# shanghong/Multiband-RF-pulse-Design

Hardware: AMD Instinct MI355X
Metric: FIR designs/sec, n=512 taps m=16384 arbitrary-phase SOCP (fir_ap_cvx form) (higher is better)
Workload: dtype f64

## Files before the change

### include/mbfir.h

```cpp
#ifndef MBFIR_H
#define MBFIR_H

#ifdef __cplusplus
extern "C" {
#endif

#define MBFIR_SOLVED 0
#define MBFIR_INFEASIBLE 1
#define MBFIR_NUMERICAL 2
#define MBFIR_EARLY_FAIL 3
#define MBFIR_E_ARG (-1)
#define MBFIR_E_HIP (-2)
#define MBFIR_E_NODEVICE (-3)

typedef struct mbfir_ctx mbfir_ctx;

typedef struct mbfir_opts {
    int grid_m;
    int max_iter;
    double feastol;
    double abstol;
    double reltol;
    int refine;
    int verbose;
// ... 3 lines not shown
    int ddkkt;
    int lanes;
} mbfir_opts;

typedef struct mbfir_info {
    int status;
    int iters;
    int n_unknowns;
    int n_rows;
    int n_freq;
    int n_lp, n_q3, n_big;
    double pcost, dcost, gap, relgap, pres, dres;
    double ms_assemble, ms_solve, ms_post, ms_total;
    double ms_gram;
    double ms_chol;
    double gram_flop;
    int gram_launches;
    int lattice;
    double chol_flop;
    int chol_launches;
    int builds;
    int dd_iters;
    int dd_kmax;
    int collectives;
    int lanes;
    int dd_form;
    double ms_cap;
    double cap_flop;
    double collective_bytes;
    int correctors;
    int correctors_taken;
    int gv_passes;
    int gtv_passes;
} mbfir_info;

typedef int (*mbfir_allreduce_fn)(void* buf, long count, int op, void* user);

int  mbfir_comm_unique_id(mbfir_ctx* ctx, char* id128);
int  mbfir_comm_init(mbfir_ctx* ctx, int nranks, int rank, const char* id128);
void mbfir_comm_destroy(mbfir_ctx* ctx);
int  mbfir_test_comm_allreduce(mbfir_ctx* ctx, double* v, long n, int op);

mbfir_ctx*  mbfir_create(int device_id);
void        mbfir_destroy(mbfir_ctx* ctx);
const char* mbfir_last_error(mbfir_ctx* ctx);
void        mbfir_default_opts(mbfir_opts* opts);
void        mbfir_set_allreduce(mbfir_ctx* ctx, mbfir_allreduce_fn fn, void* user);
const char* mbfir_version(void);

int mbfir_ap_solve(mbfir_ctx* ctx, int n, int nband, const double* f, const double* a,
                   const double* d, double obj, double peak, const mbfir_opts* opts,
                   double* h_re, double* h_im, mbfir_info* info);

int mbfir_qp_solve(mbfir_ctx* ctx, int n, int nband, const double* f, const double* a,
                   const double* d, double kquad, const double* obj, int nobj,
                   const mbfir_opts* opts, double* h_re, double* h_im, mbfir_info* info);

int mbfir_linprog_solve(mbfir_ctx* ctx, int n, int nband, const double* f, const double* a,
                        const double* d, const mbfir_opts* opts,
                        double* h_re, double* h_im, mbfir_info* info);

int mbfir_qprog_phs_solve(mbfir_ctx* ctx, int n, int nband, const double* f,
                          const double* ac_re, const double* ac_im,
                          const double* dc_re, const double* dc_im, const mbfir_opts* opts,
                          double* h_re, double* h_im, mbfir_info* info);

// ... 121 lines not shown
```

### multiband-rf-pulse-design_amd/__init__.py

```python
import ctypes as C
import os

import numpy as np

_HERE = os.path.dirname(os.path.abspath(__file__))
LIB_PATH = os.path.join(_HERE, "libmbfir.so")

SOLVED, INFEASIBLE, NUMERICAL, EARLY_FAIL = 0, 1, 2, 3
E_ARG, E_HIP, E_NODEVICE = -1, -2, -3


class MbfirError(RuntimeError):
    pass


class Opts(C.Structure):
    _fields_ = [("grid_m", C.c_int), ("max_iter", C.c_int), ("feastol", C.c_double),
                ("abstol", C.c_double), ("reltol", C.c_double), ("refine", C.c_int),
                ("verbose", C.c_int), ("shard_rank", C.c_int), ("shard_size", C.c_int),
                ("dense_trig", C.c_int), ("ddkkt", C.c_int), ("lanes", C.c_int)]


class Info(C.Structure):
    _fields_ = [("status", C.c_int), ("iters", C.c_int), ("n_unknowns", C.c_int), ("n_rows", C.c_int),
                ("n_freq", C.c_int), ("n_lp", C.c_int), ("n_q3", C.c_int), ("n_big", C.c_int),
                ("pcost", C.c_double), ("dcost", C.c_double), ("gap", C.c_double), ("relgap", C.c_double),
                ("pres", C.c_double), ("dres", C.c_double),
                ("ms_assemble", C.c_double), ("ms_solve", C.c_double), ("ms_post", C.c_double),
                ("ms_total", C.c_double), ("ms_gram", C.c_double), ("ms_chol", C.c_double),
                ("gram_flop", C.c_double), ("gram_launches", C.c_int), ("lattice", C.c_int),
                ("chol_flop", C.c_double), ("chol_launches", C.c_int), ("builds", C.c_int),
                ("dd_iters", C.c_int), ("dd_kmax", C.c_int), ("collectives", C.c_int), ("lanes", C.c_int),
                ("dd_form", C.c_int), ("ms_cap", C.c_double), ("cap_flop", C.c_double),
                ("collective_bytes", C.c_double), ("correctors", C.c_int), ("correctors_taken", C.c_int),
                ("gv_passes", C.c_int), ("gtv_passes", C.c_int)]

    def as_dict(self):
        return {k: getattr(self, k) for k, _ in self._fields_}


class Job(C.Structure):
    _fields_ = [("which", C.c_int), ("n", C.c_int), ("nband", C.c_int), ("rc", C.c_int),
                ("f", C.POINTER(C.c_double)), ("a", C.POINTER(C.c_double)), ("d", C.POINTER(C.c_double)),
                ("params", C.c_double * 4), ("h_re", C.POINTER(C.c_double)), ("h_im", C.POINTER(C.c_double)),
                ("info", Info), ("z", C.POINTER(C.c_double)), ("z_cap", C.c_int), ("err", C.c_char * 128)]


class RemezJob(C.Structure):
    _fields_ = [("numtaps", C.c_int), ("nband", C.c_int), ("type", C.c_int), ("edges", C.POINTER(C.c_double)),
                ("desired", C.POINTER(C.c_double)), ("weight", C.POINTER(C.c_double)), ("h", C.POINTER(C.c_double)),
                ("ext", C.POINTER(C.c_double)), ("status", C.c_int), ("iterations", C.c_int), ("delta", C.c_double)]


class RemezOpts(C.Structure):
    _fields_ = [("grid_density", C.c_int), ("maxiter", C.c_int)]


ALLREDUCE_FN = C.CFUNCTYPE(C.c_int, C.c_void_p, C.c_long, C.c_int, C.c_void_p)

_dp = C.POINTER(C.c_double)
_ip = C.POINTER(C.c_int)
_lp = C.POINTER(C.c_long)
_lib = None

SYMBOLS = {
    "mbfir_create": (C.c_void_p, [C.c_int]),
    "mbfir_destroy": (None, [C.c_void_p]),
    "mbfir_last_error": (C.c_char_p, [C.c_void_p]),
# ... 1119 lines not shown
```

### multiband-rf-pulse-design_amd/csrc/api.cpp

```cpp
#include "../../include/mbfir.h"
#include "program.h"
#include "pulse.h"
#include "solver.h"
#include <chrono>
#include <cmath>
#include <cstdio>
#include <algorithm>
#include <cstdlib>
#include <cstring>
#include <functional>
#include <atomic>
#include <condition_variable>
#include <map>
#include <mutex>
#include <memory>
#include <system_error>
#include <thread>

using namespace mbfir;

struct mbfir_ctx {
    std::unique_ptr<Solver> solver;
    int device = 0;
    std::vector<double> last_x;
// ... 30 lines not shown
    s.shard_size = o->shard_size;
    s.dense_trig = o->dense_trig != 0;
    return s;
}

int status_to_rc(int st) {
    switch (st) {
        case ST_OPTIMAL:
        case ST_OPTIMAL_INACCURATE: return MBFIR_SOLVED;
        case ST_PRIMAL_INFEASIBLE:
        case ST_DUAL_INFEASIBLE: return MBFIR_INFEASIBLE;
        default: return MBFIR_NUMERICAL;
    }
}

void fill_info(mbfir_info* info, const TrigProgram& P, const SolveInfo& si, int rc, double t0, double t_asm,
               double t_solved, double t_end) {
    if (!info) return;
    std::memset(info, 0, sizeof(*info));
    info->status = rc; info->iters = si.iters; info->n_unknowns = P.N();
    info->n_rows = si.n_rows; info->n_freq = si.n_freq;
    info->n_lp = P.l; info->n_q3 = P.nq3; info->n_big = P.big;
    info->pcost = si.pcost; info->dcost = si.dcost; info->gap = si.gap; info->relgap = si.relgap;
    info->pres = si.pres; info->dres = si.dres;
    info->ms_assemble = (t_asm - t0) + si.ms_assemble; info->ms_solve = si.ms_solve;
    info->ms_post = t_end - t_solved; info->ms_total = t_end - t0;
    info->ms_gram = si.ms_gram; info->ms_chol = si.ms_chol; info->gram_flop = si.gram_flop;
    info->gram_launches = si.lattice ? 0 : si.h_builds * (P.quad ? 3 : 1);
    info->lattice = si.lattice;
    info->chol_launches = si.chol_launches; info->chol_flop = si.chol_flop; info->builds = si.h_builds;
    info->dd_iters = si.dd_iters; info->dd_kmax = si.dd_kmax; info->lanes = si.lanes; info->collectives = si.collectives;
    info->collective_bytes = si.collective_bytes;
    info->ms_cap = si.ms_cap; info->cap_flop = si.cap_flop; info->dd_form = si.dd_iters > 0 ? si.dd_form : -1;
    info->correctors = si.correctors; info->correctors_taken = si.correctors_taken; info->gv_passes = si.gv_passes; info->gtv_passes = si.gtv_passes;
}

void taps_from_solution(Solver& solver, const TrigProgram& P, const std::vector<double>& x, int lane, double* h_re, double* h_im) {
    const int n = P.n;
    switch (P.which) {
        case DES_AP:
            solver.specfact_last(n, h_re, h_im, lane);
            break;
        case DES_LINPROG: {
            const int nh = P.nhalf;
            for (int i = 0; i < n; ++i) { h_re[i] = 0; h_im[i] = 0; }
            if (P.real_filter) {
                if (P.odd_filter) for (int k = 0; k < nh; ++k) { h_re[nh - 1 + k] = x[k]; h_re[nh - 1 - k] = x[k]; }
                else for (int k = 0; k < nh; ++k) { h_re[nh + k] = x[k]; h_re[nh - 1 - k] = x[k]; }
            } else if (P.odd_filter) {
                for (int k = 0; k < nh; ++k) {
                    double re = x[k], im = k == 0 ? 0.0 : x[nh + k - 1];
                    h_re[nh - 1 + k] = re; h_im[nh - 1 + k] = im;
                    h_re[nh - 1 - k] = re; h_im[nh - 1 - k] = -im;
                }
            } else {
                for (int k = 0; k < nh; ++k) {
                    double re = x[k], im = x[nh + k];
                    h_re[nh + k] = re; h_im[nh + k] = im;
                    h_re[nh - 1 - k] = re; h_im[nh - 1 - k] = -im;
                }
            }
            break;
        }
        default:
            for (int i = 0; i < n; ++i) { h_re[i] = x[i]; h_im[i] = x[n + i]; }
    }
}
// ... 832 lines not shown
```

### multiband-rf-pulse-design_amd/csrc/solver.h

```cpp
#pragma once
#include "program.h"
#include <stdexcept>
#include <string>
#include <vector>

namespace mbfir {

struct ShapeError : std::runtime_error {
    explicit ShapeError(const std::string& s) : std::runtime_error(s) {}
};
struct ResourceError : std::runtime_error {
    explicit ResourceError(const std::string& s) : std::runtime_error(s) {}
};

enum { ST_OPTIMAL = 0, ST_PRIMAL_INFEASIBLE = 1, ST_DUAL_INFEASIBLE = 2, ST_MAXIT = 3, ST_NUMERICAL = 4,
       ST_OPTIMAL_INACCURATE = 5 };

struct SolveOpts {
    int max_iter = 200;
    double feastol = 1e-8, abstol = 1e-10, reltol = 1e-8;
    int refine = 2;
    int verbose = 0;
    int shard_rank = 0, shard_size = 1;
    bool dense_trig = false;
    double ddkkt_theta = 0;
    int dd_form = 0;
    bool timing = true;
};

struct SolveInfo {
    int status = 0, iters = 0, n_unknowns = 0, n_rows = 0, n_freq = 0;
    double pcost = 0, dcost = 0, gap = 0, relgap = 0, pres = 0, dres = 0;
    double ms_assemble = 0, ms_solve = 0, ms_gram = 0, ms_chol = 0, gram_flop = 0;
    int h_builds = 0;
    int chol_launches = 0;
    double chol_flop = 0;
    int dd_iters = 0, dd_kmax = 0;
    double ms_cap = 0, cap_flop = 0;
    int dd_form = 0;
    int collectives = 0;
    double collective_bytes = 0;
    int lanes = 1;
    int lattice = 0;
    int correctors = 0, correctors_taken = 0;
    int gv_passes = 0, gtv_passes = 0;
};

class Solver {
public:
    explicit Solver(int device);
    ~Solver();
    Solver(const Solver&) = delete;
    Solver& operator=(const Solver&) = delete;
    int solve(const TrigProgram& P, const SolveOpts& o, std::vector<double>& xout, SolveInfo& info);
    void solve_lanes(const std::vector<const TrigProgram*>& Ps, const SolveOpts& o, std::vector<std::vector<double>>& xouts,
                     std::vector<SolveInfo>& infos);
    static std::vector<long> shape_key(const TrigProgram& P, const SolveOpts& o);
    static int max_lanes(const TrigProgram& P, const SolveOpts& o);
    static void test_fold(const double* w, int Mf, int fold, long* out);
    void specfact_last(int n, double* h_re, double* h_im, int lane = 0);
    void set_solution(const std::vector<double>& x);
    void test_gram(int m, int nt, int nw, const double* A, const double* d, double* out);
    void test_chol(int n, const double* H, double* out_l, double* out_m);
    void test_chol_lanes(int n, int nlanes, int form, const int* mask, const double* H, double* out_l, double* out_m);
    void test_specfact(int n, const double* x, double* h_re, double* h_im);
    void test_ddsolve(int n, int k, const double* H, const double* U, const double* X, int nrhs, const double* bh,
                      const double* bl, double* xh, double* xl, int* nfix, double* Lh_out = nullptr, double* Ll_out = nullptr);
    void test_mfma_peak(double* tf_mfma, double* tf_valu);
    void test_time_kernels(int n, int m, int nt, int reps, double* ms_chol, double* ms_gram);
    void* stream() const;
    void comm_unique_id(char* id128);
    void comm_init(int nranks, int rank, const char* id128);
    void comm_destroy();
    void test_comm_allreduce(double* v, long n, int op);
    void set_allreduce(int (*fn)(void*, long, int, void*), void* user);

private:
// ... 6 lines not shown
```

### multiband-rf-pulse-design_amd/csrc/solver.hip

```cpp
#include "dev_common.h"
#include <functional>
#include <mutex>
#include <thread>
#include "cone_dev.h"
#include "dd_dev.h"
#include "program.h"
#include "solver.h"
#include <algorithm>
#include <chrono>
#include <cmath>
#include <cstdlib>
#include <cstring>
#include <vector>

#include <dlfcn.h>
#include <rccl/rccl.h>

namespace mbfir {

struct RcclApi {
    ncclResult_t (*GetUniqueId)(ncclUniqueId*) = nullptr;
    ncclResult_t (*CommInitRank)(ncclComm_t*, int, ncclUniqueId, int) = nullptr;
    ncclResult_t (*CommDestroy)(ncclComm_t) = nullptr;
    ncclResult_t (*AllReduce)(const void*, void*, size_t, ncclDataType_t, ncclRedOp_t, ncclComm_t, hipStream_t) = nullptr;
// ... 474 lines not shown
            if (P.quad) {
                const double c2 = qj >= 0 ? qs * vin[(long)q * P.LDV + qj] : 0.0;
                if (kind) cf[NV + q][e >> 1].y = c2; else cf[NV + q][e >> 1].x = c2;
            }
        }
    }
    __syncthreads();
    if (k >= P.nfold) return;
    const double4 sd4 = P.seed_eval[(long)sg * P.Mpad + k];
    double c = sd4.x, s = sd4.y;
    const double cw = sd4.z, sw = sd4.w;
    double ac[NVVMAX], as[NVVMAX];
#pragma unroll
    for (int v = 0; v < NVVMAX; ++v) ac[v] = as[v] = 0;
#pragma unroll 8
    for (int m = 0; m < m1 - m0; ++m) {
#pragma unroll
        for (int v = 0; v < NVVMAX; ++v)
            if (v < NVV) { const double2 x = cf[v][m]; ac[v] += x.x * c; as[v] += x.y * s; }
        const double cn = c * cw - s * sw;
        s = s * cw + c * sw;
        c = cn;
    }
    const int ip = P.fold_pos[k], in = P.fold_neg[k];
#pragma unroll
    for (int v = 0; v < NVVMAX; ++v)
        if (v < NVV) {
            double* u = UU + ((long)sg * NVV + v) * P.Mpad;
            if (ip >= 0) u[ip] = ac[v] + as[v];
            if (in >= 0) u[in] = ac[v] - as[v];
        }
}

__global__ void k_build_seeds_m(DProg P, double ka, int na, double kb, int nb, double4* __restrict__ seeds) {
    LANES(P, seeds);
    if (P.dims) { na = P.D1; nb = nb ? 2 * P.D1 - 1 : 0; }
    const double t0a = ka * P.tmin, t0b = kb * P.tmin;
    const int m = blockIdx.x * blockDim.x + threadIdx.x, ch = blockIdx.y;
    if (m >= na + nb || ch >= P.nchunk) return;
    const double t = m < na ? t0a + m : t0b + (m - na);
    double s, c, sd, cd;
    sincos(P.ch_w0[ch] * t, &s, &c);
    sincos(P.ch_dw[ch] * t, &sd, &cd);
    seeds[(long)ch * (na + nb) + m] = make_double4(c, s, cd, sd);
}
__global__ void k_build_seeds_e(DProg P, double4* __restrict__ seeds) {
    LANES(P, seeds);
    const int i = blockIdx.x * blockDim.x + threadIdx.x, sg = blockIdx.y;
    if (i >= P.nfold) return;
    const double w = P.wf[i];
    double s, c, sw, cw;
    sincos(w * (P.tmin + sg * P.seg), &s, &c);
    sincos(w, &sw, &cw);
    seeds[(long)sg * P.Mpad + i] = make_double4(c, s, cw, sw);
}

constexpr int CGRP = 4;
constexpr int MPTS = 256;
template <int NV, bool AGG>
__device__ __forceinline__ void freq_operands(const DProg& P, const double* __restrict__ src, int i, double (&out)[NV]) {
#pragma unroll
    for (int v = 0; v < NV; ++v) out[v] = 0;
    if (i < 0) return;
    if (AGG) {
        const int nv = P.quad ? NV / 2 : NV;
        for (int qq = P.f_ptr[i]; qq < P.f_ptr[i + 1]; ++qq) {
// ... 49 lines not shown
    }
    __syncthreads();
    const int m = blockIdx.x * MPTS + tid;
    if (m >= na + nb) return;
    double ag[NV], as[NV];
#pragma unroll
    for (int v = 0; v < NV; ++v) ag[v] = as[v] = 0;
    for (int cl = 0; cl < P.cgrp; cl += 2) {
        const int cha = ch0 + cl, chb = cha + 1;
        if (cha >= P.nchunk) break;
        const bool two = cl + 1 < P.cgrp && chb < P.nchunk;
        const double4 sa = seeds[(long)cha * (na + nb) + m];
        const double4 sb = two ? seeds[(long)chb * (na + nb) + m] : make_double4(0.0, 0.0, 0.0, 0.0);
        double c0 = sa.x, s0 = sa.y, c1 = sb.x, s1 = sb.y;
        const int cnt = max(P.ch_count[cha], two ? P.ch_count[chb] : 0);
        const int clb = two ? cl + 1 : cl;
#pragma unroll 4
        for (int q = 0; q < cnt; ++q) {
#pragma unroll
            for (int v = 0; v < NV; ++v) {
                const double2 pa = pp[v][cl][q], pb = pp[v][clb][q];
                ag[v] += pa.x * c0; as[v] += pa.y * s0;
                ag[v] += pb.x * c1; as[v] += pb.y * s1;
            }
            const double n0 = c0 * sa.z - s0 * sa.w, n1 = c1 * sb.z - s1 * sb.w;
            s0 = s0 * sa.z + c0 * sa.w; s1 = s1 * sb.z + c1 * sb.w;
            c0 = n0; c1 = n1;
        }
    }
#pragma unroll
    for (int v = 0; v < NV; ++v) {
        partial[(((long)blockIdx.y * NV + v) * 2) * P.LDM + m] = ag[v];
        partial[(((long)blockIdx.y * NV + v) * 2 + 1) * P.LDM + m] = as[v];
    }
}

template <int NC>
__device__ __forceinline__ void block_partials(double vals[NC], double* __restrict__ part, bool is_max) {
    __shared__ double sh[17];
#pragma unroll
    for (int c = 0; c < NC; ++c) {
        double s = is_max ? block_max(vals[c], sh) : block_sum(vals[c], sh);
        if (threadIdx.x == 0) part[(long)blockIdx.x * NC + c] = s;
    }
}
__device__ __forceinline__ double fold_partials(const double* part, int nb, int nc, int c, bool is_max, double* sh) {
    double a = is_max ? -1e300 : 0.0;
    for (int b = threadIdx.x; b < nb; b += blockDim.x) {
        double v = part[(long)b * nc + c];
        a = is_max ? fmax(a, v) : a + v;
    }
    return is_max ? block_max(a, sh) : block_sum(a, sh);
}

struct BigW {
    double eta, w0;
};
__device__ __forceinline__ double big_dot(const double* a, const double* b, int n, double* sh) {
    double t = 0;
    for (int i = threadIdx.x; i < n; i += blockDim.x) t += a[i] * b[i];
    return block_sum(t, sh);
}

__global__ __launch_bounds__(1024) void k_big_scaling(DProg P, const double* __restrict__ s,
                                                      const double* __restrict__ z, double* __restrict__ wbb,
                                                      double* __restrict__ lam, double* __restrict__ Sc) {
// ... 1120 lines not shown
__global__ void k_unit_scaling(DProg P, double* __restrict__ dl, double* __restrict__ wl, double* __restrict__ w3,
                               double* __restrict__ wbb, double* __restrict__ Sc) {
    LANES(P, dl, wl, w3, wbb, Sc);
    int t = blockIdx.x * blockDim.x + threadIdx.x;
    if (t < P.l) { dl[t] = 1.0; wl[t] = 1.0; }
    if (t < P.nq3) { w3[4 * t] = 1.0; w3[4 * t + 1] = 1.0; w3[4 * t + 2] = 0.0; w3[4 * t + 3] = 0.0; }
    if (t < P.big) wbb[t] = t == 0 ? 1.0 : 0.0;
    if (t == 0) { Sc[S_ETAB] = 1.0; Sc[S_WB0] = 1.0; }
}
__global__ void k_finish_x(DProg P, const double* __restrict__ x, const double* __restrict__ Sc, double* __restrict__ out) {
    LANES(P, x, Sc, out);
    int j = blockIdx.x * blockDim.x + threadIdx.x;
    if (j < P.N) out[j] = x[j] / Sc[S_TAU];
}
#include "ddkkt.inc"

struct SolveSwitches {
    bool corrector = true;
    bool corr_big = true;
    int test_cap_kp = 0;
    int ar_chunks = 0;
    int ar_overlap = 1;
    int cgrp = 4;
    int ddform = -1;
    bool dd_blockinv = true;
    bool hsolve = true;
    bool fuse = true;
    bool speculate = true;
    bool trace_host = false;
    int fold = -1;
    int chol_split = -1;
    bool poison = false;
    int test_lose_flag = -1;
};
static SolveSwitches read_switches() {
    SolveSwitches w;
    auto flag = [](const char* name, bool& v) { if (const char* ev = std::getenv(name)) v = std::atoi(ev) != 0; };
    auto number = [](const char* name, int& v) { if (const char* ev = std::getenv(name)) v = std::atoi(ev); };
    flag("MBFIR_CORRECTOR", w.corrector); flag("MBFIR_CORR_BIG", w.corr_big); flag("MBFIR_DD_BLOCKINV", w.dd_blockinv);
    flag("MBFIR_HSOLVE", w.hsolve); flag("MBFIR_FUSE", w.fuse); flag("MBFIR_SPECULATE", w.speculate); flag("MBFIR_POISON", w.poison);
    number("MBFIR_TEST_CAP_KP", w.test_cap_kp); number("MBFIR_AR_OVERLAP", w.ar_overlap);
    number("MBFIR_CHOL_SPLIT", w.chol_split); number("MBFIR_TEST_LOSE_FLAG", w.test_lose_flag);
    if (const char* ev = std::getenv("MBFIR_CGRP")) w.cgrp = std::max(1, std::min(CGRP, std::atoi(ev)));
    if (const char* ev = std::getenv("MBFIR_AR_CHUNKS")) w.ar_chunks = std::max(1, std::atoi(ev));
    if (const char* ev = std::getenv("MBFIR_DDFORM")) w.ddform = std::strcmp(ev, "dd") != 0 ? 1 : 0;
    if (const char* ev = std::getenv("MBFIR_FOLD")) w.fold = std::atoi(ev) != 0;
    w.trace_host = std::getenv("MBFIR_TRACE_HOST") != nullptr;
    return w;
}

struct LatticeInfo {
    bool ok = false;
    double tmin = 0;
    int D1 = 0;
    std::vector<int> lat, lat_col, lat_qcol, ch_start, ch_count;
    std::vector<double> lat_scale, lat_qscale, ch_w0, ch_dw;
    std::vector<int> fold_pos, fold_neg;
    std::vector<double> wf;
};
constexpr int CHUNK_LEN = 64;
static_assert(CHUNK_LEN <= CHK, "a chunk holds at most CHK frequencies");
static LatticeInfo analyse_lattice(const TrigProgram& Q, bool fold) {
    LatticeInfo L;
    const int Nt = Q.Nt, Mf = Q.Mf;
    if (Nt <= 0 || Mf <= 0) return L;
    double tmin = Q.col_tau[0];
    for (double t : Q.col_tau) tmin = std::min(tmin, t);
    L.lat.resize(Nt);
    int D1 = 0;
    for (int j = 0; j < Nt; ++j) {
        const double m = Q.col_tau[j] - tmin;
        const long mi = std::lround(m);
        if (std::fabs(m - double(mi)) > 1e-9 || mi > 8L * Nt + 64) return L;
// ... 186 lines not shown
    if (L.first_opt >= 0 && it >= L.first_opt + POLISH_MAX) return finish(ST_OPTIMAL);
    {
        const bool approach = finite && (hs[S_GAP] <= POLISH_APPROACH * o.abstol || hs[S_RELGAP] <= POLISH_APPROACH * o.reltol);
        L.nsweep = std::min(MAX_SWEEPS, L.nsweep_ctl + ((approach || L.first_opt >= 0) ? POLISH_SWEEPS : 0));
    }
    if (!finite) return finish(ST_NUMERICAL);
    const bool collapsed = hs[S_KAPPA] / hs[S_TAU] >= 1e6;
    if (L.first_opt < 0 && (hs[S_PINF] <= o.feastol || (collapsed && hs[S_PINF] <= 1e-5))) return finish(ST_PRIMAL_INFEASIBLE);
    if (L.first_opt < 0 && (hs[S_DINF] <= o.feastol || (collapsed && hs[S_DINF] <= 1e-5))) return finish(ST_DUAL_INFEASIBLE);
    if (L.first_opt < 0 && hs[S_PRES] <= INACC_FEAS && hs[S_DRES] <= INACC_FEAS) {
        double merit = std::min(hs[S_RELGAP], hs[S_GAP] / std::max(o.abstol, 1e-300) * o.reltol);
        if (merit < L.best_merit) {
            L.best_merit = merit; L.best_info = info; L.have_best = true;
            best = true;
        }
    }
    if (it == o.max_iter) return finish(ST_MAXIT);
    L.wall = (int(hs[S_CHOLFIX]) > 0 && (hs[S_PRES] > INACC_FEAS || hs[S_DRES] > INACC_FEAS)) ? L.wall + 1 : 0;
    if (L.wall >= WALL_ITERS) return finish(ST_NUMERICAL);
    return best;
}

struct Solver::Impl {
    int device = 0;
    hipStream_t st = nullptr;
    int shard_rank = 0, shard_size = 1;
    int (*ar_fn)(void*, long, int, void*) = nullptr;
    void* ar_user = nullptr;
    double* RB = nullptr;
    ncclComm_t comm = nullptr;
    int comm_size = 0, comm_rank = 0;
    long n_collectives = 0;
    double collective_bytes = 0;
    long n_gv = 0, n_gtv = 0;
    void allreduce(double* buf, long count, int op, hipStream_t on = nullptr) {
        if (shard_size <= 1) return;
        if (!on) on = st;
        ++n_collectives;
        collective_bytes += 8.0 * double(count);
        if (comm) {
            ncclResult_t r = rccl().AllReduce(buf, buf, size_t(count), ncclDouble, op == 1 ? ncclMax : ncclSum, comm, on);
            if (r != ncclSuccess) throw HipError(std::string("ncclAllReduce: ") + (rccl().GetErrorString ? rccl().GetErrorString(r) : "failed"));
            return;
        }
        MBFIR_HIP(hipStreamSynchronize(on));
        if (!ar_fn || ar_fn(buf, count, op, ar_user) != 0) throw HipError("all-reduce hook failed");
    }
    hipEvent_t ev0 = nullptr, ev1 = nullptr;
    Arena ar;
    double* hostSc = nullptr;
    int* hostFlag = nullptr;
    int nlanes = 1, nlanes_last = 1;
    bool taps_valid = false;
    int lane_n[64] = {};
    long chol_launch_count = 0;
    size_t lane_bytes = 0;
    bool lane_live[64] = {};
    bool fused_hsolve = false;
    int* maskT = nullptr;
    int* hostMask = nullptr;
    LaneDims* dimsT = nullptr;
    LaneDims* hostDims = nullptr;
    const int* mask_row(int r) const { return nlanes > 1 ? maskT + (size_t)r * MAX_LANES : nullptr; }
    std::string err;

    DProg P{};
// ... 86 lines not shown
                    if (q.bytes) {
                        size_t nb = 0;
                        const void* src = q.src(b, nb);
                        if (nb > q.bytes) nb = q.bytes;
                        if (nb) std::memcpy(img + (q.off - stage_lo), src, nb);
                        if (nb < q.bytes) std::memset(img + (q.off - stage_lo) + nb, 0, q.bytes - nb);
                    }
                }
                const size_t filled = stage_hi - stage_lo;
                if (region > filled) std::memset(img + filled, 0, region - filled);
                rc[t] = hipMemcpyAsync(ar.base + stage_lo + (size_t)b * lane_bytes, img, region, hipMemcpyHostToDevice, st);
            }
        };
        std::vector<std::thread> th;
        for (int t = 1; t < nth; ++t) th.emplace_back(fill, t);
        fill(0);
        for (auto& t : th) t.join();
        for (hipError_t e : rc) MBFIR_HIP(e);
        pend.clear();
        stage_lo = stage_hi = 0;
    }
    void memset_lanes(void* p, size_t bytes) {
        if ((bytes & 15) == 0 && (reinterpret_cast<size_t>(p) & 15) == 0 && (lane_bytes & 15) == 0)
            hipLaunchKernelGGL(k_zero_lanes, dim3(std::min<size_t>(2048, cdiv((long)(bytes / 16), 256)), nlanes), dim3(256), 0, st,
                               reinterpret_cast<double2*>(p), bytes / 16, lane_bytes);
        else if (nlanes > 1) hipMemset2DAsync(p, lane_bytes, 0, bytes, nlanes, st);
        else hipMemsetAsync(p, 0, bytes, st);
    }
    void copy_lanes(void* dst, const void* src, size_t bytes) {
        if (nlanes > 1) MBFIR_HIP(hipMemcpy2DAsync(dst, lane_bytes, src, lane_bytes, bytes, nlanes, hipMemcpyDeviceToDevice, st));
        else MBFIR_HIP(hipMemcpyAsync(dst, src, bytes, hipMemcpyDeviceToDevice, st));
    }

    template <int NV>
    void apply_G(const double* v, double* out) {
        const int NVV = P.quad ? 2 * NV : NV;
        ++n_gv;
        if (P.trig) {
            hipLaunchKernelGGL(k_trig_eval<NV>, lane_grid(dim3(cdiv(P.nfold, 256), P.useg), nlanes), dim3(256), 0, st, P, v, UU);
            hipLaunchKernelGGL(k_rows_G<NV>, lane_grid(dim3(cdiv(P.R, 256)), nlanes), dim3(256), 0, st, P, UU, v, out);
            return;
        }
        const double* xx = v;
        if (P.quad) {
            hipLaunchKernelGGL(k_make_xx<NV>, lane_grid(dim3(cdiv(P.Nt, 256)), nlanes), dim3(256), 0, st, P, v, XX);
            xx = XX;
        }
        dim3 g(cdiv(P.Mf, 4));
        if (NVV == 1) hipLaunchKernelGGL(k_amulti<1>, lane_grid(g, nlanes), dim3(256), 0, st, A1, P.ld, P.Mf, xx, P.LDV, UU, P.Mpad, lane_bytes, P.mask, P.dims);
        else if (NVV == 2) hipLaunchKernelGGL(k_amulti<2>, lane_grid(g, nlanes), dim3(256), 0, st, A1, P.ld, P.Mf, xx, P.LDV, UU, P.Mpad, lane_bytes, P.mask, P.dims);
        else hipLaunchKernelGGL(k_amulti<4>, lane_grid(g, nlanes), dim3(256), 0, st, A1, P.ld, P.Mf, xx, P.LDV, UU, P.Mpad, lane_bytes, P.mask, P.dims);
        hipLaunchKernelGGL(k_rows_G<NV>, lane_grid(dim3(cdiv(P.R, 256)), nlanes), dim3(256), 0, st, P, UU, v, out);
    }
    template <int NV>
    void apply_G_winv2(const double* v, double* gout, const double* sub, double* wout) {
        if (P.trig && !P.big) {
            ++n_gv;
            hipLaunchKernelGGL(k_trig_eval<NV>, lane_grid(dim3(cdiv(P.nfold, 256), P.useg), nlanes), dim3(256), 0, st, P, v, UU);
            hipLaunchKernelGGL(k_rows_winv2<NV>, lane_grid(dim3(cdiv(P.l + P.nq3, 256)), nlanes), dim3(256), 0, st, P, UU, v, dl, w3, sub, gout, wout);
            return;
        }
        apply_G<NV>(v, gout);
        winv2<NV>(gout, sub, wout, 0);
    }
    void moments_array(int nv, const double* pp, const double4* seeds, int na, int nb, double* out) {
        dim3 g(cdiv(na + nb, MPTS), cdiv(P.nchunk, P.cgrp)), b(256), gf(cdiv(P.nfold, 256));
        switch (nv) {
#define MOM_CASE(NVX)                                                                                                          \
            case NVX:                                                                                                          \
                if (pp) hipLaunchKernelGGL((k_freq_fold<NVX, false>), lane_grid(gf, nlanes), b, 0, st, P, pp, PPf);            \
                hipLaunchKernelGGL((k_trig_moments<NVX>), lane_grid(g, nlanes), b, 0, st, P, PPf, seeds, na, nb, partial);     \
                break;
            MOM_CASE(1) MOM_CASE(2) MOM_CASE(3) MOM_CASE(4) MOM_CASE(6)
#undef MOM_CASE
            default: throw HipError("moments: unsupported vector count");
        }
        hipLaunchKernelGGL(k_fold_partials, lane_grid(dim3(cdiv(P.LDM, 64), 2 * nv), nlanes), dim3(64, 16), 0, st, partial, cdiv(P.nchunk, P.cgrp), 2 * nv, P.LDM, P.LDM, out, lane_bytes, P.mask, P.dims, P.cgrp);
    }
    void atmulti_array(int nvv, const double* pp) {
        dim3 g(P.ld / 128, nsplit_at), b(64, 4);
        switch (nvv) {
            case 1: hipLaunchKernelGGL((k_atmulti<1, false>), lane_grid(g, nlanes), b, 0, st, P, A1, pp, partial); break;
            case 2: hipLaunchKernelGGL((k_atmulti<2, false>), lane_grid(g, nlanes), b, 0, st, P, A1, pp, partial); break;
            case 3: hipLaunchKernelGGL((k_atmulti<3, false>), lane_grid(g, nlanes), b, 0, st, P, A1, pp, partial); break;
            case 4: hipLaunchKernelGGL((k_atmulti<4, false>), lane_grid(g, nlanes), b, 0, st, P, A1, pp, partial); break;
            case 6: hipLaunchKernelGGL((k_atmulti<6, false>), lane_grid(g, nlanes), b, 0, st, P, A1, pp, partial); break;
            default: throw HipError("atmulti: unsupported vector count");
        }
    }
    template <int NV>
    void apply_GT(const double* val, double* out, int tail = 0, const double* rn_bx = nullptr, double* rn_r = nullptr, int rn_slot = 0) {
        ++n_gtv;
        if (P.trig) {
            dim3 g(cdiv(P.D1, MPTS), cdiv(P.nchunk, P.cgrp)), b(256);
            const dim3 gf(cdiv(P.nfold, 256));
            if (sw.fuse) {
                if (P.quad) hipLaunchKernelGGL((k_trig_moments<2 * NV, true>), lane_grid(g, nlanes), b, 0, st, P, (const double2*)nullptr, P.seed_tau, P.D1, 0, partial, val);
                else hipLaunchKernelGGL((k_trig_moments<NV, true>), lane_grid(g, nlanes), b, 0, st, P, (const double2*)nullptr, P.seed_tau, P.D1, 0, partial, val);
            } else if (P.quad) {
                hipLaunchKernelGGL((k_freq_fold<2 * NV, true>), lane_grid(gf, nlanes), b, 0, st, P, val, PPf);
                hipLaunchKernelGGL((k_trig_moments<2 * NV>), lane_grid(g, nlanes), b, 0, st, P, PPf, P.seed_tau, P.D1, 0, partial);
            } else {
                hipLaunchKernelGGL((k_freq_fold<NV, true>), lane_grid(gf, nlanes), b, 0, st, P, val, PPf);
                hipLaunchKernelGGL((k_trig_moments<NV>), lane_grid(g, nlanes), b, 0, st, P, PPf, P.seed_tau, P.D1, 0, partial);
            }
        } else {
            dim3 g(P.ld / 128, nsplit_at), b(64, 4);
            if (P.quad) hipLaunchKernelGGL((k_atmulti<2 * NV, true>), lane_grid(g, nlanes), b, 0, st, P, A1, val, partial);
            else hipLaunchKernelGGL((k_atmulti<NV, true>), lane_grid(g, nlanes), b, 0, st, P, A1, val, partial);
        }
        hipLaunchKernelGGL(k_gt_finish<NV>, lane_grid(dim3(cdiv(P.Nt, GTC) + 1), nlanes), dim3(GTC, GTG), 0, st, P, partial, P.trig ? cdiv(P.nchunk, P.cgrp) : nsplit_at, val, out,
                           GtResid{rn_bx, rn_r, Sc, rn_slot, gt_cnt});
        allreduce(out, (long)NV * P.LDV + tail, 0);
    }
    template <int NV>
    void winv2(const double* in, const double* sub, double* out, int mode) {
        hipLaunchKernelGGL(k_winv2<NV>, lane_grid(dim3(cdiv(P.l + P.nq3, 256)), nlanes), dim3(256), 0, st, P, dl, w3, in, sub, out, mode);
        if (P.big) hipLaunchKernelGGL(k_big_winv2<NV>, lane_grid(dim3(1), nlanes), dim3(1024), 0, st, P, wbb, Sc, in, sub, out, mode);
    }
    bool lead_factor() const { return shard_size > 1 && P.trig; }
    int* gt_cnt = nullptr;
    template <int NV>
    void hsolve(const double* rhs, double* out, const double* rhs2 = nullptr) {
        if (fused_hsolve) {
            hsolve_launch(M, P.np, rhs, rhs2, out, partial, NV, P.LDV, st, nlanes, lane_bytes, P.mask);
        } else {
            trigemv_launch(M, P.np, 0, rhs, yN, NV, P.LDV, st, rhs2, nlanes, lane_bytes, P.mask);
            trigemv_launch(Mt, P.np, 1, yN, out, NV, P.LDV, st, nullptr, nlanes, lane_bytes, P.mask);
        }
// ... 274 lines not shown
        P.dd_lane = nullptr; P.dl_plain = nullptr;
        if (ddk > 0 && cap_form) {
            const int kp = dd_unit ? dd_kp : std::max(int(round_up(ddk, 64)), sw.test_cap_kp);
            const size_t lb = dd_unit ? lane_bytes : 0;
            const int* mdd = mask_row(ROW_DD);
            chol_launch_count += chol_inv_launch(H, M, fused_hsolve ? nullptr : Mt, W1, P.np, flag, st, sw.chol_split, sw.poison, nullptr, c0, nullptr, nlanes, lb, P.mask);
            P.mask = mdd;
            hipLaunchKernelGGL(k_dd_rows, lane_grid(dim3(kp), nlanes), dim3(256), 0, st, P, D, P.np, dd_unit ? -1 : ddk);
            P.mask = live_mask;
            hipEvent_t b0 = timing ? next_cap_event() : nullptr, b1 = timing ? next_cap_event() : nullptr;
            if (b0) hipEventRecord(b0, st);
            cap_build_launch(D.U, dd_unit ? kp : ddk, kp, P.np, M, D.sX, capYt, capZt, capS, capPart, st, nlanes, lb, mdd, dd_unit ? D.kcnt : nullptr);
            if (b1) hipEventRecord(b1, st);
            cap_flop_sum += 2.0 * (double(kp) * P.np * P.np + 0.5 * double(kp) * kp * P.np);
            chol_inv_launch(capS, capMs, nullptr, capW1, kp, capflag, st, sw.chol_split, sw.poison, nullptr, nullptr, c1, nlanes, lb, mdd);
            cap_flag_add_launch(flag, capflag, st, nlanes, lb, mdd);
        } else if (ddk > 0) {
            if (c0) hipEventRecord(c0, st);
            hipLaunchKernelGGL(k_dd_rows, lane_grid(dim3(ddk), nlanes), dim3(256), 0, st, P, D, P.np, ddk);
            dd_syrk_launch(D.U, P.np, D.sX, D.kcnt, P.np, H, M, st);
            dd_chol_launch(H, M, Mt, W1, ddri, ddri + P.np, ddd0, P.np, DD_PIVTOL, flag, st, ddinv);
            if (c1) hipEventRecord(c1, st);
        } else {
            chol_launch_count += chol_inv_launch(H, M, fused_hsolve ? nullptr : Mt, W1, P.np, flag, st, sw.chol_split, sw.poison, nullptr, c0, c1, nlanes, lane_bytes, P.mask);
        }
    }
    void prepare_lanes(const std::vector<const TrigProgram*>& Qs, const SolveOpts& o, std::vector<LaneHost>& LH) {
        shard_rank = o.shard_size > 1 ? o.shard_rank : 0;
        shard_size = o.shard_size > 1 ? o.shard_size : 1;
        if (shard_size > 1 && !ar_fn && !comm) throw HipError("row-sharded solve without a communicator or an all-reduce hook");
        if (comm && shard_size > 1 && (comm_size != shard_size || comm_rank != shard_rank))
            throw HipError("row-sharded solve: shard_rank / shard_size differ from the RCCL communicator's");
        n_collectives = 0; collective_bytes = 0;
        n_gv = 0; n_gtv = 0;
        if (shard_size > 1 && nlanes > 1) throw ShapeError("row-sharded solves run one design at a time");
        for (int b = 0; b < nlanes; ++b) {
            LaneHost& L = LH[b];
            const TrigProgram& Qfull = *Qs[b];
            if (shard_size > 1) { L.local = shard_program(Qfull, shard_rank, shard_size); L.Q = &L.local; }
            else L.Q = &Qfull;
            double nh = 0, nc = 0;
            for (double v : Qfull.h) nh += v * v;
            for (double v : Qfull.c) nc += v * v;
            L.nrm_h = std::max(1.0, std::sqrt(nh)); L.nrm_c = std::max(1.0, std::sqrt(nc));
            L.degree = double(Qfull.l + Qfull.nq3 + (Qfull.big ? 1 : 0));
            L.prep = lane_prep(*L.Q, o, sw);
            L.Lt = L.prep->Lt;
            L.nsweep = o.refine; L.nsweep_ctl = o.refine;
        }
        if (shard_size > 1 && !o.dense_trig) {
            ensure_arena(4096);
            double* dv = reinterpret_cast<double*>(ar.base);
            hostSc[0] = LH[0].Lt.ok ? -1.0 : 0.0;
            MBFIR_HIP(hipMemcpyAsync(dv, hostSc, sizeof(double), hipMemcpyHostToDevice, st));
            allreduce(dv, 1, 1);
            MBFIR_HIP(hipMemcpyAsync(hostSc, dv, sizeof(double), hipMemcpyDeviceToHost, st));
            MBFIR_HIP(hipStreamSynchronize(st));
            if (hostSc[0] > -0.5) LH[0].Lt = LatticeInfo();
        }
    }
    UnitPlan plan_unit(const std::vector<LaneHost>& LH, const SolveOpts& o) {
        const TrigProgram& Q = *LH[0].Q;
        const LatticeInfo& Lt = LH[0].Lt;
        int Mf_max = Q.Mf, R_max = Q.R, l_max = Q.l, nyrows_max = int(LH[0].prep->yrows.size());
        int Nt_max = Q.Nt, nq3_max = Q.nq3, big_max = Q.big, D1_max = Lt.D1, n_max = Q.n;
        size_t nchunk_max = Lt.ch_start.size(), nfold_max = Lt.wf.size();
        bool hetero = false, orders = false;
// ... 404 lines not shown
                const int keep_it = L.info.iters;
                L.info = L.best_info; L.info.iters = keep_it;
                L.status = ST_OPTIMAL_INACCURATE;
                MBFIR_HIP(hipMemcpyAsync(xo, reinterpret_cast<char*>(xbest) + (size_t)b * lane_bytes, sizeof(double) * P.LDV, hipMemcpyDeviceToDevice, st));
            }
            const int Nb = L.Q->N();
            xouts[b].assign(Nb, 0.0);
            MBFIR_HIP(hipMemcpyAsync(xouts[b].data(), xo, sizeof(double) * Nb, hipMemcpyDeviceToHost, st));
        }
        MBFIR_HIP(hipStreamSynchronize(st));
        const double t_end = now_ms();
        double ms_gram = 0, ms_chol = 0;
        int builds = 0;
        for (size_t i = 0; i + 3 < evused; i += 4, ++builds) {
            float a = 0, b = 0;
            if (hipEventElapsedTime(&a, evpool[i], evpool[i + 1]) == hipSuccess) ms_gram += a;
            if (hipEventElapsedTime(&b, evpool[i + 2], evpool[i + 3]) == hipSuccess) ms_chol += b;
        }
        double ms_cap = 0;
        for (size_t i = 0; i + 1 < capev_used; i += 2) { float t = 0; hipEventElapsedTime(&t, capev[i], capev[i + 1]); ms_cap += t; }
        const int nw = P.quad ? 3 : 1;
        for (int b = 0; b < nlanes; ++b) {
            SolveInfo& info = infos[b];
            info = LH[b].info;
            info.status = LH[b].status;
            info.ms_assemble = t_assembled - t_begin;
            info.ms_solve = t_end - t_assembled;
            info.ms_gram = ms_gram; info.ms_chol = ms_chol; info.h_builds = builds;
            info.n_freq = LH[b].Q->Mf; info.n_rows = LH[b].Q->R; info.n_unknowns = LH[b].Q->N();
            info.lattice = P.trig;
            info.lanes = nlanes;
            info.collectives = int(n_collectives);
            info.collective_bytes = collective_bytes;
            info.gv_passes = int(n_gv); info.gtv_passes = int(n_gtv);
            info.dd_iters = LH[b].dd_iters; info.dd_kmax = LH[b].dd_kmax;
            info.dd_form = cap_form ? 0 : 1; info.cap_flop = cap_flop_sum; info.ms_cap = ms_cap;
            info.chol_launches = int(chol_launch_count);
            info.chol_flop = 2.0 / 3.0 * double(P.np) * double(P.np) * double(P.np);
            info.gram_flop = P.trig ? double(3 * P.D1 - 1) * double(LH[b].Q->Mf) * (4.0 + 4.0 * nw)
                                    : double(nw) * double(P.Mf) * double(P.Nt) * double(P.Nt + 1);
        }
        nlanes_last = nlanes; taps_valid = false;
    }
};

Solver::Solver(int device) : impl(new Impl()) {
    impl->device = device;
    int ndev = 0;
    if (hipGetDeviceCount(&ndev) != hipSuccess || ndev <= 0) throw HipError("no HIP device available");
    MBFIR_HIP(hipSetDevice(device));
    {
        static std::mutex warm_mu;
        static std::vector<char> warmed;
        std::lock_guard<std::mutex> lk(warm_mu);
        if (device < 0 || device >= ndev) throw HipError("no such HIP device");
        if ((int)warmed.size() < ndev) warmed.resize(ndev, 0);
        if (!warmed[device]) { dd_warm_kernels(); chol_warm_kernels(); warmed[device] = 1; }
    }
    MBFIR_HIP(hipStreamCreate(&impl->st));
    MBFIR_HIP(hipEventCreate(&impl->ev0));
    MBFIR_HIP(hipEventCreate(&impl->ev1));
    MBFIR_HIP(hipHostMalloc(&impl->hostSc, sizeof(double) * S_COUNT * MAX_LANES));
    MBFIR_HIP(hipHostMalloc(&impl->hostFlag, sizeof(int) * 4 * MAX_LANES));
    MBFIR_HIP(hipHostMalloc(&impl->hostMask, sizeof(int) * MASK_ROWS * MAX_LANES));
    MBFIR_HIP(hipMalloc(&impl->maskT, sizeof(int) * MASK_ROWS * MAX_LANES));
    MBFIR_HIP(hipMalloc(&impl->dimsT, sizeof(LaneDims) * MAX_LANES));
    MBFIR_HIP(hipHostMalloc(&impl->hostDims, sizeof(LaneDims) * MAX_LANES));
// ... 487 lines not shown
```

Baseline: 301.5.

## Process two design lanes per block in trig eval and moments kernels

Adds paired-lane variants of the trigonometric evaluation and moment kernels, where each block handles two batched designs that share frequency seeds. Each block then reuses the seed loads and rotation recurrences across both lanes and launches half as many lane blocks. The paths are on by default when there are at least two lanes, seeds are shared, the solve is unsharded and the fused path is selected. In exchange they double shared memory and register pressure per block, which may lower occupancy, and they add a pair_passes counter to the info struct.

```diff
diff --git a/include/mbfir.h b/include/mbfir.h
--- a/include/mbfir.h
+++ b/include/mbfir.h
@@ -59,6 +59,7 @@
     int correctors_taken;
     int gv_passes;
     int gtv_passes;
+    int pair_passes;
 } mbfir_info;
 
 typedef int (*mbfir_allreduce_fn)(void* buf, long count, int op, void* user);
diff --git a/multiband-rf-pulse-design_amd/__init__.py b/multiband-rf-pulse-design_amd/__init__.py
--- a/multiband-rf-pulse-design_amd/__init__.py
+++ b/multiband-rf-pulse-design_amd/__init__.py
@@ -33,7 +33,7 @@
                 ("dd_iters", C.c_int), ("dd_kmax", C.c_int), ("collectives", C.c_int), ("lanes", C.c_int),
                 ("dd_form", C.c_int), ("ms_cap", C.c_double), ("cap_flop", C.c_double),
                 ("collective_bytes", C.c_double), ("correctors", C.c_int), ("correctors_taken", C.c_int),
-                ("gv_passes", C.c_int), ("gtv_passes", C.c_int)]
+                ("gv_passes", C.c_int), ("gtv_passes", C.c_int), ("pair_passes", C.c_int)]
 
     def as_dict(self):
         return {k: getattr(self, k) for k, _ in self._fields_}
diff --git a/multiband-rf-pulse-design_amd/csrc/api.cpp b/multiband-rf-pulse-design_amd/csrc/api.cpp
--- a/multiband-rf-pulse-design_amd/csrc/api.cpp
+++ b/multiband-rf-pulse-design_amd/csrc/api.cpp
@@ -86,7 +86,7 @@
     info->dd_iters = si.dd_iters; info->dd_kmax = si.dd_kmax; info->lanes = si.lanes; info->collectives = si.collectives;
     info->collective_bytes = si.collective_bytes;
     info->ms_cap = si.ms_cap; info->cap_flop = si.cap_flop; info->dd_form = si.dd_iters > 0 ? si.dd_form : -1;
-    info->correctors = si.correctors; info->correctors_taken = si.correctors_taken; info->gv_passes = si.gv_passes; info->gtv_passes = si.gtv_passes;
+    info->correctors = si.correctors; info->correctors_taken = si.correctors_taken; info->gv_passes = si.gv_passes; info->gtv_passes = si.gtv_passes; info->pair_passes = si.pair_passes;
 }
 
 void taps_from_solution(Solver& solver, const TrigProgram& P, const std::vector<double>& x, int lane, double* h_re, double* h_im) {
diff --git a/multiband-rf-pulse-design_amd/csrc/solver.h b/multiband-rf-pulse-design_amd/csrc/solver.h
--- a/multiband-rf-pulse-design_amd/csrc/solver.h
+++ b/multiband-rf-pulse-design_amd/csrc/solver.h
@@ -43,6 +43,7 @@
     int lanes = 1;
     int lattice = 0;
     int correctors = 0, correctors_taken = 0;
+    int pair_passes = 0;
     int gv_passes = 0, gtv_passes = 0;
 };
 
diff --git a/multiband-rf-pulse-design_amd/csrc/solver.hip b/multiband-rf-pulse-design_amd/csrc/solver.hip
--- a/multiband-rf-pulse-design_amd/csrc/solver.hip
+++ b/multiband-rf-pulse-design_amd/csrc/solver.hip
@@ -530,6 +530,100 @@
         }
 }
 
+template <int SFUSE>
+__device__ __forceinline__ void rotate(double& c, double& s, double cd, double sd) {
+    const double cn = fma(c, cd, -(s * sd));
+    s = SFUSE ? fma(c, sd, s * cd) : fma(s, cd, c * sd);
+    c = cn;
+}
+__device__ __forceinline__ bool pair_prologue(DProg& P, int nlanes, bool (&live)[2], size_t& off0) {
+    const int l0 = 2 * blockIdx.z;
+    live[0] = !P.mask || P.mask[l0];
+    live[1] = l0 + 1 < nlanes && (!P.mask || P.mask[l0 + 1]);
+    off0 = (size_t)l0 * P.lane_bytes;
+    if (!live[0] && !live[1]) return false;
+    if (l0) P.shift(off0);
+    return true;
+}
+template <class T>
+__device__ __forceinline__ T* byte_shift(T* p, size_t off) { return (T*)((const char*)p + off); }
+template <int NVVMAX, int NL, int NVC>
+__device__ __forceinline__ void trig_eval_sum(const double2 (*cf)[NVVMAX][SEGMAX], int n, int NVV, const double4 sd4, double (&ac)[NL][NVVMAX], double (&as)[NL][NVVMAX]) {
+    double c = sd4.x, s = sd4.y;
+    const double cw = sd4.z, sw = sd4.w;
+#pragma unroll
+    for (int L = 0; L < NL; ++L)
+#pragma unroll
+    for (int v = 0; v < NVVMAX; ++v) ac[L][v] = as[L][v] = 0;
+#pragma unroll (8 / NL)
+    for (int m = 0; m < n; ++m) {
+#pragma unroll
+        for (int L = 0; L < NL; ++L)
+#pragma unroll
+        for (int v = 0; v < NVVMAX; ++v)
+            if (NVC ? v < NVC : v < NVV) { const double2 x = cf[L][v][m]; ac[L][v] += x.x * c; as[L][v] += x.y * s; }
+        rotate<0>(c, s, cw, sw);
+    }
+}
+template <int NV, int NL>
+__device__ __forceinline__ void trig_eval_lanes(const DProg& P, const double* const (&vin)[NL], double* const (&UU)[NL], double2 (*cf)[2 * NV][SEGMAX]) {
+    constexpr int NVVMAX = 2 * NV;
+    const int k = blockIdx.x * 256 + threadIdx.x, sg = blockIdx.y;
+    const int m0 = sg * P.seg, m1 = min(m0 + P.seg, P.D1);
+    const int NVV = P.quad ? 2 * NV : NV;
+    for (int e = threadIdx.x; e < 2 * (m1 - m0); e += 256) {
+        const int kind = e & 1, m = m0 + (e >> 1), le = kind * P.D1 + m;
+        const int j = P.lat_col[le], qj = P.quad ? P.lat_qcol[le] : -1;
+        const double sc = P.lat_scale[le], qs = P.quad ? P.lat_qscale[le] : 0.0;
+#pragma unroll
+        for (int L = 0; L < NL; ++L)
+#pragma unroll
+        for (int q = 0; q < NV; ++q) {
+            const double c1 = j >= 0 ? sc * vin[L][(long)q * P.LDV + j] : 0.0;
+            if (kind) cf[L][q][e >> 1].y = c1; else cf[L][q][e >> 1].x = c1;
+            if (P.quad) {
+                const double c2 = qj >= 0 ? qs * vin[L][(long)q * P.LDV + qj] : 0.0;
+                if (kind) cf[L][NV + q][e >> 1].y = c2; else cf[L][NV + q][e >> 1].x = c2;
+            }
+        }
+    }
+    __syncthreads();
+    if (k >= P.nfold) return;
+    const double4 sd4 = P.seed_eval[(long)sg * P.Mpad + k];
+    double ac[NL][NVVMAX], as[NL][NVVMAX];
+    if (NL == 1) trig_eval_sum<NVVMAX, NL, 0>(cf, m1 - m0, NVV, sd4, ac, as);
+    else if (P.quad) trig_eval_sum<NVVMAX, NL, NVVMAX>(cf, m1 - m0, NVV, sd4, ac, as);
+    else trig_eval_sum<NVVMAX, NL, NV>(cf, m1 - m0, NVV, sd4, ac, as);
+    const int ip = P.fold_pos[k], in = P.fold_neg[k];
+#pragma unroll
+    for (int L = 0; L < NL; ++L)
+#pragma unroll
+    for (int v = 0; v < NVVMAX; ++v)
+        if (v < NVV) {
+            double* u = UU[L] + ((long)sg * NVV + v) * P.Mpad;
+            if (ip >= 0) u[ip] = ac[L][v] + as[L][v];
+            if (in >= 0) u[in] = ac[L][v] - as[L][v];
+        }
+}
+template <int NV>
+__global__ __launch_bounds__(256, 8) void k_trig_eval_pair(DProg P, const double* __restrict__ vin, double* __restrict__ UU, int nlanes) {
+    __shared__ double2 cf[2][2 * NV][SEGMAX];
+    bool live[2];
+    size_t off0;
+    if (!pair_prologue(P, nlanes, live, off0)) return;
+    const bool both = live[0] && live[1];
+    const size_t off1 = (both || !live[0]) ? P.lane_bytes : 0;
+    if (both) {
+        const double* const v2[2] = {byte_shift(vin, off0), byte_shift(vin, off0 + off1)};
+        double* const u2[2] = {byte_shift(UU, off0), byte_shift(UU, off0 + off1)};
+        trig_eval_lanes<NV, 2>(P, v2, u2, cf);
+    } else {
+        const double* const v1[1] = {byte_shift(vin, off0 + off1)};
+        double* const u1[1] = {byte_shift(UU, off0 + off1)};
+        trig_eval_lanes<NV, 1>(P, v1, u1, cf);
+    }
+}
+
 __global__ void k_build_seeds_m(DProg P, double ka, int na, double kb, int nb, double4* __restrict__ seeds) {
     LANES(P, seeds);
     if (P.dims) { na = P.D1; nb = nb ? 2 * P.D1 - 1 : 0; }
@@ -645,6 +739,90 @@
     for (int v = 0; v < NV; ++v) {
         partial[(((long)blockIdx.y * NV + v) * 2) * P.LDM + m] = ag[v];
         partial[(((long)blockIdx.y * NV + v) * 2 + 1) * P.LDM + m] = as[v];
+    }
+}
+
+template <int NV, int NL>
+__device__ __forceinline__ void trig_moments_lanes(const DProg& P, const DProg* const (&PL)[NL], const double4* __restrict__ seeds, int na,
+                                                   double* const (&partial)[NL], const double* const (&rows)[NL], double2 (*pp)[NV][CGRP][CHK]) {
+    constexpr int nb = 0;
+    const int tid = threadIdx.x;
+    const int ch0 = blockIdx.y * P.cgrp;
+    for (int e = tid; e < P.cgrp * CHK; e += 256) {
+        const int cc = e / CHK, q = e - cc * CHK, ch = ch0 + cc;
+        const bool live = ch < P.nchunk && q < P.ch_count[ch < P.nchunk ? ch : 0];
+        const int k = live ? P.ch_start[ch] + q : 0;
+        const int kp = live ? P.fold_pos[k] : -1, kn = live ? P.fold_neg[k] : -1;
+#pragma unroll
+        for (int L = 0; L < NL; ++L) {
+            double a[NV], b[NV];
+            freq_operands<NV, true>(*PL[L], rows[L], kp, a);
+            freq_operands<NV, true>(*PL[L], rows[L], kn, b);
+#pragma unroll
+            for (int v = 0; v < NV; ++v) pp[L][v][cc][q] = make_double2(a[v] + b[v], a[v] - b[v]);
+        }
+    }
+    __syncthreads();
+    const int m = blockIdx.x * MPTS + tid;
+    if (m >= na + nb) return;
+    double ag[NL][NV], as[NL][NV];
+#pragma unroll
+    for (int L = 0; L < NL; ++L)
+#pragma unroll
+    for (int v = 0; v < NV; ++v) ag[L][v] = as[L][v] = 0;
+    for (int cl = 0; cl < P.cgrp; cl += 2) {
+        const int cha = ch0 + cl, chb = cha + 1;
+        if (cha >= P.nchunk) break;
+        const bool two = cl + 1 < P.cgrp && chb < P.nchunk;
+        const double4 sa = seeds[(long)cha * (na + nb) + m];
+        const double4 sb = two ? seeds[(long)chb * (na + nb) + m] : make_double4(0.0, 0.0, 0.0, 0.0);
+        double c0 = sa.x, s0 = sa.y, c1 = sb.x, s1 = sb.y;
+        const int cnt = max(P.ch_count[cha], two ? P.ch_count[chb] : 0);
+        const int clb = two ? cl + 1 : cl;
+#pragma unroll (4 / NL)
+        for (int q = 0; q < cnt; ++q) {
+#pragma unroll
+            for (int L = 0; L < NL; ++L)
+#pragma unroll
+            for (int v = 0; v < NV; ++v) {
+                const double2 pa = pp[L][v][cl][q], pb = pp[L][v][clb][q];
+                ag[L][v] += pa.x * c0; as[L][v] += pa.y * s0;
+                ag[L][v] += pb.x * c1; as[L][v] += pb.y * s1;
+            }
+            rotate<1>(c0, s0, sa.z, sa.w);
+            rotate<1>(c1, s1, sb.z, sb.w);
+        }
+    }
+#pragma unroll
+    for (int L = 0; L < NL; ++L)
+#pragma unroll
+    for (int v = 0; v < NV; ++v) {
+        partial[L][(((long)blockIdx.y * NV + v) * 2) * P.LDM + m] = ag[L][v];
+        partial[L][(((long)blockIdx.y * NV + v) * 2 + 1) * P.LDM + m] = as[L][v];
+    }
+}
+template <int NV>
+__global__ __launch_bounds__(256, 8) void k_trig_moments_pair(DProg P, const double4* __restrict__ seeds, int na, double* __restrict__ partial,
+                                                              const double* __restrict__ rows, int nlanes) {
+    static_assert(NV <= 2, "k_trig_moments_pair: one or two operands");
+    __shared__ double2 pp[2][NV][CGRP][CHK];
+    bool live[2];
+    size_t off0;
+    if (!pair_prologue(P, nlanes, live, off0)) return;
+    const bool both = live[0] && live[1];
+    const size_t off1 = (both || !live[0]) ? P.lane_bytes : 0;
+    DProg Q = P;
+    Q.shift(off1);
+    if (both) {
+        const DProg* const p2[2] = {&P, &Q};
+        double* const o2[2] = {byte_shift(partial, off0), byte_shift(partial, off0 + off1)};
+        const double* const r2[2] = {byte_shift(rows, off0), byte_shift(rows, off0 + off1)};
+        trig_moments_lanes<NV, 2>(P, p2, seeds, na, o2, r2, pp);
+    } else {
+        const DProg* const p1[1] = {&Q};
+        double* const o1[1] = {byte_shift(partial, off0 + off1)};
+        const double* const r1[1] = {byte_shift(rows, off0 + off1)};
+        trig_moments_lanes<NV, 1>(P, p1, seeds, na, o1, r1, pp);
     }
 }
 
@@ -1831,6 +2009,7 @@
     int chol_split = -1;
     bool poison = false;
     int test_lose_flag = -1;
+    bool lanepair = true;
 };
 static SolveSwitches read_switches() {
     SolveSwitches w;
@@ -1838,6 +2017,7 @@
     auto number = [](const char* name, int& v) { if (const char* ev = std::getenv(name)) v = std::atoi(ev); };
     flag("MBFIR_CORRECTOR", w.corrector); flag("MBFIR_CORR_BIG", w.corr_big); flag("MBFIR_DD_BLOCKINV", w.dd_blockinv);
     flag("MBFIR_HSOLVE", w.hsolve); flag("MBFIR_FUSE", w.fuse); flag("MBFIR_SPECULATE", w.speculate); flag("MBFIR_POISON", w.poison);
+    flag("MBFIR_LANEPAIR", w.lanepair);
     number("MBFIR_TEST_CAP_KP", w.test_cap_kp); number("MBFIR_AR_OVERLAP", w.ar_overlap);
     number("MBFIR_CHOL_SPLIT", w.chol_split); number("MBFIR_TEST_LOSE_FLAG", w.test_lose_flag);
     if (const char* ev = std::getenv("MBFIR_CGRP")) w.cgrp = std::max(1, std::min(CGRP, std::atoi(ev)));
@@ -2090,6 +2270,7 @@
     int comm_size = 0, comm_rank = 0;
     long n_collectives = 0;
     double collective_bytes = 0;
+    long n_pair = 0;
     long n_gv = 0, n_gtv = 0;
     void allreduce(double* buf, long count, int op, hipStream_t on = nullptr) {
         if (shard_size <= 1) return;
@@ -2242,12 +2423,21 @@
         else MBFIR_HIP(hipMemcpyAsync(dst, src, bytes, hipMemcpyDeviceToDevice, st));
     }
 
+    bool lane_pairs() const { return sw.lanepair && nlanes >= 2 && P.seeds_shared && !P.dims && shard_size == 1 && !dd_unit; }
+    template <int NV>
+    void trig_eval(const double* v) {
+        const dim3 g(cdiv(P.nfold, 256), P.useg);
+        if (lane_pairs()) {
+            ++n_pair;
+            hipLaunchKernelGGL(k_trig_eval_pair<NV>, lane_grid(g, cdiv(nlanes, 2)), dim3(256), 0, st, P, v, UU, nlanes);
+        } else hipLaunchKernelGGL(k_trig_eval<NV>, lane_grid(g, nlanes), dim3(256), 0, st, P, v, UU);
+    }
     template <int NV>
     void apply_G(const double* v, double* out) {
         const int NVV = P.quad ? 2 * NV : NV;
         ++n_gv;
         if (P.trig) {
-            hipLaunchKernelGGL(k_trig_eval<NV>, lane_grid(dim3(cdiv(P.nfold, 256), P.useg), nlanes), dim3(256), 0, st, P, v, UU);
+            trig_eval<NV>(v);
             hipLaunchKernelGGL(k_rows_G<NV>, lane_grid(dim3(cdiv(P.R, 256)), nlanes), dim3(256), 0, st, P, UU, v, out);
             return;
         }
@@ -2266,7 +2456,7 @@
     void apply_G_winv2(const double* v, double* gout, const double* sub, double* wout) {
         if (P.trig && !P.big) {
             ++n_gv;
-            hipLaunchKernelGGL(k_trig_eval<NV>, lane_grid(dim3(cdiv(P.nfold, 256), P.useg), nlanes), dim3(256), 0, st, P, v, UU);
+            trig_eval<NV>(v);
             hipLaunchKernelGGL(k_rows_winv2<NV>, lane_grid(dim3(cdiv(P.l + P.nq3, 256)), nlanes), dim3(256), 0, st, P, UU, v, dl, w3, sub, gout, wout);
             return;
         }
@@ -2304,7 +2494,13 @@
         if (P.trig) {
             dim3 g(cdiv(P.D1, MPTS), cdiv(P.nchunk, P.cgrp)), b(256);
             const dim3 gf(cdiv(P.nfold, 256));
-            if (sw.fuse) {
+            constexpr bool PAIR1 = NV <= 2, PAIR2 = 2 * NV <= 2;
+            if (sw.fuse && lane_pairs() && (P.quad ? PAIR2 : PAIR1)) {
+                const dim3 g2 = lane_grid(g, cdiv(nlanes, 2));
+                ++n_pair;
+                if constexpr (PAIR2) if (P.quad) hipLaunchKernelGGL(k_trig_moments_pair<2 * NV>, g2, b, 0, st, P, P.seed_tau, P.D1, partial, val, nlanes);
+                if constexpr (PAIR1) if (!P.quad) hipLaunchKernelGGL(k_trig_moments_pair<NV>, g2, b, 0, st, P, P.seed_tau, P.D1, partial, val, nlanes);
+            } else if (sw.fuse) {
                 if (P.quad) hipLaunchKernelGGL((k_trig_moments<2 * NV, true>), lane_grid(g, nlanes), b, 0, st, P, (const double2*)nullptr, P.seed_tau, P.D1, 0, partial, val);
                 else hipLaunchKernelGGL((k_trig_moments<NV, true>), lane_grid(g, nlanes), b, 0, st, P, (const double2*)nullptr, P.seed_tau, P.D1, 0, partial, val);
             } else if (P.quad) {
@@ -2645,7 +2841,7 @@
         if (comm && shard_size > 1 && (comm_size != shard_size || comm_rank != shard_rank))
             throw HipError("row-sharded solve: shard_rank / shard_size differ from the RCCL communicator's");
         n_collectives = 0; collective_bytes = 0;
-        n_gv = 0; n_gtv = 0;
+        n_gv = 0; n_gtv = 0; n_pair = 0;
         if (shard_size > 1 && nlanes > 1) throw ShapeError("row-sharded solves run one design at a time");
         for (int b = 0; b < nlanes; ++b) {
             LaneHost& L = LH[b];
@@ -3116,7 +3312,7 @@
             info.lanes = nlanes;
             info.collectives = int(n_collectives);
             info.collective_bytes = collective_bytes;
-            info.gv_passes = int(n_gv); info.gtv_passes = int(n_gtv);
+            info.gv_passes = int(n_gv); info.gtv_passes = int(n_gtv); info.pair_passes = int(n_pair);
             info.dd_iters = LH[b].dd_iters; info.dd_kmax = LH[b].dd_kmax;
             info.dd_form = cap_form ? 0 : 1; info.cap_flop = cap_flop_sum; info.ms_cap = ms_cap;
             info.chol_launches = int(chol_launch_count);
```

Measured after the change: 307.5, median of 6. +2.0%, better.
